# SiddhantSKarki/Vision-Transformer

Measured on AMD Instinct MI355X. Metric: images/sec fwd+bwd ViT-Base/16 224^2 bf16 (train step incl. AdamW); % MFMA roofline, higher is better.
Workload: dtype bf16; 1 GPU; ViT-Base/16 224x224 train step (fwd+CE+bwd+AdamW), batch 256/GPU; model=vit_base_patch16_224, global_batch=256, seq_len=197, parallelism=dp1

## Files before the change

include/vit_hip.h:

```cpp
#ifndef VIT_HIP_H
#define VIT_HIP_H

#include <stdint.h>

#ifdef __cplusplus
extern "C" {
#endif

#define VIT_ABI_VERSION 18

typedef enum { VIT_OK = 0, VIT_ERR_INVALID = 1, VIT_ERR_LAUNCH = 2 } vit_status;
typedef enum { VIT_F32 = 0, VIT_BF16 = 1, VIT_MASK4 = 2 } vit_dtype;

typedef enum { VIT_ACT_NONE = 0, VIT_ACT_RELU = 1, VIT_ACT_GELU = 2 } vit_act;

#define VIT_FLAG_SHARED_CUS 1

int vit_abi_version(void);
const char* vit_last_error(void);

int vit_set_option(const char* name, int64_t value);
int64_t vit_get_option(const char* name);

typedef struct vit_gemm_desc {
  const void* a;
  const void* b;
  void* c;
  int64_t lda, ldb, ldc;
  int64_t m, n, k;
  int32_t a_kcontig, b_kcontig;
  int32_t in_dtype;
  int32_t out_dtype;
  float alpha, beta;
  const float* bias;
  int32_t act;
  int32_t aux_dtype;
  const void* aux;
  int64_t ldaux;
  const void* res;
  int64_t ldres;
  int64_t res_rowmod;
  int32_t res_dtype;
  float dropout_p;
  uint32_t dropout_seed;
  int32_t split_k;
  int64_t out_group_rows, out_group_stride;
  void* workspace;
  int64_t workspace_bytes;
  float* colsum_part;
  void* mask_out;
  int64_t dropout_row_stride;
  int32_t flags;
  int64_t dropout_row0;
} vit_gemm_desc;

int64_t vit_gemm_workspace_bytes(const vit_gemm_desc* d);
int vit_gemm_split_k_hint(int64_t m, int64_t n, int64_t k, int in_dtype);
int vit_gemm(const vit_gemm_desc* d, void* stream);

#define VIT_DROP_PATH_MAX_LAYERS 64
int vit_drop_path_rows(float* out, uint32_t seed, int64_t L, int64_t B, int64_t T, const float* rates ,
                       void* stream);
int vit_gemm_rowscale(const vit_gemm_desc* d, const float* row_scale , void* stream);

#define VIT_EPI_BDR 3
#define VIT_EPI_SLAB 4
#define VIT_EPI_GENERAL 5
#define VIT_EPI_BDRS 8
int vit_gemm_kernel_choice(const vit_gemm_desc* d, const float* row_scale, int32_t* impl, int32_t* kind);

int vit_im2col(const void* x, int32_t x_dtype, void* cols, int32_t dtype, int64_t B, int64_t C, int64_t H,
               int64_t W, int64_t P, void* stream);
int vit_col2im(const void* cols, int32_t dtype, void* x, int32_t x_dtype, int64_t B, int64_t C, int64_t H, int64_t W,
               int64_t P, void* stream);
int vit_embed_cls(const float* cls, const float* pos, void* x0, int32_t dtype, int64_t B, int64_t T, int64_t D,
                  void* stream);

int vit_layernorm_fwd(const void* x, int64_t ldx, const float* gamma, const float* beta, void* y, int64_t ldy,
                      float* mean, float* rstd, int64_t rows, int64_t cols, float eps, int32_t dtype, void* stream);
int64_t vit_layernorm_bwd_parts(int64_t rows, int64_t cols);
int vit_layernorm_bwd(const void* dy, int64_t lddy, const void* x, int64_t ldx, const float* gamma,
                      const float* mean, const float* rstd, const void* dres, void* dx_out, void* drop_out,
                      float drop_p, uint32_t drop_seed, const void* drop_mask, float* partial, int32_t osum,
                      int64_t rows, int64_t cols, int32_t dtype, void* stream);

int vit_attn_fwd(const void* qkv, void* o, float* o32, float* lse, float* probs, int64_t B, int64_t T, int64_t H,
                 int64_t hd, float scale, int32_t dtype, int64_t max_wgs, void* stream);
int vit_attn_bwd_uses_o32(int64_t B, int64_t T, int64_t H, int64_t hd, int32_t dtype);
int64_t vit_attn_bwd_workspace_bytes(int64_t B, int64_t T, int64_t H, int64_t hd, int32_t dtype);
int vit_attn_bwd(const void* qkv, const void* o, const float* o32, const void* d_o, const float* lse, void* dqkv,
                 int64_t B, int64_t T, int64_t H, int64_t hd, float scale, int32_t dtype, void* workspace,
                 int32_t flags, void* stream);

int vit_attn_fwd_row0(const void* qkv, void* o, float* lse, int64_t B, int64_t T, int64_t H, int64_t hd, float scale,
                      int32_t dtype, void* stream);
int vit_attn_bwd_row0(const void* qkv, const void* d_o0, int64_t ldo, void* dqkv, int64_t B, int64_t T, int64_t H,
                      int64_t hd, float scale, int32_t dtype, void* stream);

int64_t vit_colsum_workspace_bytes(int64_t rows, int64_t cols);
int vit_colsum(const void* x, int64_t ldx, int32_t dtype, int64_t rows, int64_t cols, float* out, float alpha,
               float beta, void* workspace, void* stream);
int vit_colsum_finish(const float* part, int64_t nparts, int64_t cols, int32_t nsets, float* out0, float* out1,
                      float* out2, float beta, void* stream);
typedef struct {
  const float* part;
  int64_t nparts, cols;
  int32_t nsets;
  float* out[3];
  float beta;
} vit_colsum_job;
int vit_colsum_finish_batch(const vit_colsum_job* jobs, int32_t njobs, void* stream);
int vit_copy2d(const void* src, int64_t lds, int32_t src_dtype, void* dst, int64_t ldd, int32_t dst_dtype,
               int64_t rows, int64_t cols, int64_t src_group_rows, int64_t src_group_stride, float beta,
               void* stream);
int vit_dropout_bwd(const void* x, void* y, int32_t dtype, int64_t n, float p, uint32_t seed, float scale,
                    void* stream);
int vit_relu_bwd(const void* dy, const void* y, void* dx, int32_t dtype, int64_t n, void* stream);
// ... 80 lines not shown
```

vision-transformer_amd/VisionTransformer/_engine.py:

```python
from __future__ import annotations

import contextlib
import ctypes
import math
import weakref
from typing import NamedTuple, Optional

import torch
import torch.distributed as dist
from torch.optim.optimizer import register_optimizer_step_post_hook
from torch.utils.weak import WeakIdKeyDictionary

from . import _lib, _ops
from ._ops import ACT_NONE, ACT_RELU

SHADOWS = WeakIdKeyDictionary()


def shadow_of(p):
    return SHADOWS.get(p)


_ENGINE_OF = {}

# ... 15 lines not shown

DROPOUT_P = 0.2
LN_EPS = 1e-5
ALIGN = 64


def _hash_u32(seed, idx):
    x = (idx * 0x9E3779B1 + seed) & 0xFFFFFFFF
    x ^= x >> 16
    x = (x * 0x85EBCA6B) & 0xFFFFFFFF
    x ^= x >> 13
    x = (x * 0xC2B2AE35) & 0xFFFFFFFF
    x ^= x >> 16
    return x


def site_seed(base_seed, layer, site):
    return _hash_u32((base_seed * 0x632BE5AB + 0x1234567) & 0xFFFFFFFF, layer * 2 + site)


def dropout_seed(base_seed, rank=0):
    if rank == 0:
        return base_seed
    return _hash_u32((base_seed ^ 0x5BD1E995) & 0xFFFFFFFF, 0x27D4EB2F + rank) & 0x7FFFFFFF


def path_keep(base_seed, L, layer, site, B, p):
    thr = min(int(ctypes.c_float(p).value * 4294967296.0), 0xFFFFFFFF)
    s = site_seed(base_seed, L + layer, site)
    return torch.tensor([_hash_u32(s, b) >= thr for b in range(B)], dtype=torch.bool)


def _keep_scale(p):
    if p == 0.0:
        return DROPOUT_P, 1.0 / (1.0 - DROPOUT_P)
    keep = (1.0 - DROPOUT_P) * (1.0 - p)
    return 1.0 - keep, 1.0 / keep


class _Region:
    def __init__(self):
        self.size = 0
        self.items = []

    def add(self, name, numel):
        off = self.size
        self.items.append((name, off, numel))
        self.size = off + ((numel + ALIGN - 1) // ALIGN) * ALIGN
        return off


def split_k_for(m, n, k, dtype=torch.bfloat16):
    return int(_lib.load().vit_gemm_split_k_hint(m, n, k, _ops.dtype_code(dtype)))


def head_split_for(m, n, k):
    tiles = ((m + 63) // 64) * ((n + 63) // 64)
    nkt = (k + 31) // 32
    return max(1, min((1024 + tiles - 1) // tiles, nkt // 4, 32))


class Tape:
    __slots__ = ("B", "cols", "blocks", "z", "u", "gz", "zn", "mh", "rh", "seed", "training", "x_shape", "x_dtype",
                 "x_grad", "pruned", "row0", "path_rates")


BLOCK_REGIONS = ("qkv_w", "proj_w", "proj_b", "fc1_w", "fc1_b", "fc2_w", "fc2_b", "ln1_w", "ln1_b", "ln2_w", "ln2_b")


class BlockActs(NamedTuple):
    x_in: torch.Tensor
    a1: torch.Tensor
    m1: torch.Tensor
    r1: torch.Tensor
    qkv: torch.Tensor
    o: torch.Tensor
    o32: Optional[torch.Tensor]
    lse: torch.Tensor
    x_mid: torch.Tensor
    a2: torch.Tensor
    m2: torch.Tensor
    r2: torch.Tensor
    h: torch.Tensor
    hm: Optional[torch.Tensor]
    pm: Optional[torch.Tensor]
    fm: Optional[torch.Tensor]

    def images(self, b0, B, T):
        r0, R = b0 * T, B * T
        D = self.x_mid.shape[1]

        def rows(t):
            return None if t is None else t[r0:r0 + R]

        def bits(mask, n):
            if mask is None:
                return None
            off = (r0 // 4) * ((n + 3) // 4) * 4
            return mask[off:off + _ops.mask4_bytes(R, n)]

        s = self
        return BlockActs(x_in=rows(s.x_in), a1=rows(s.a1), m1=rows(s.m1), r1=rows(s.r1), qkv=rows(s.qkv), o=rows(s.o),
                         o32=rows(s.o32), lse=s.lse[b0:b0 + B], x_mid=rows(s.x_mid), a2=rows(s.a2), m2=rows(s.m2),
                         r2=rows(s.r2), h=rows(s.h), hm=bits(s.hm, 4 * D), pm=bits(s.pm, D), fm=bits(s.fm, D))


# ... 177 lines not shown
        self.stats["packs"] += 1

    def _token_rows(self, name, M, D, dt, T, dev):
        key = (name, M, D, dt, T, dev)
        buf = self._tok.get(key) if self._tok is not None else None
        if buf is None:
            if self._tok is None:
                self._tok = {}
            buf = self._tok[key] = torch.zeros(M, D, dtype=dt, device=dev)
        return buf

    def _workspace(self, nbytes, side=False):
        ws = self._ws[side]
        if ws is None or ws.numel() * 4 < nbytes:
            ws = self._ws[side] = torch.empty(max(nbytes // 4 + 1, 1 << 20), dtype=torch.float32, device=self.device)
        return ws

    def _split_ws(self, split, m, n, side=False):
        return self._workspace(split * m * n * 4, side) if split > 1 else None

    def _side_stream(self):
        if not self.concurrent_wgrad or self.device is None or self.device.type != "cuda":
            return None
        if self._wstream is None or self._wstream.device != self.device:
            self._wstream = torch.cuda.Stream(device=self.device)
        return self._wstream

    def _mark(self, fam, phase, flop=0.0, nbytes=0.0):
        h = self.profile_hook
        if h is not None:
            h(fam, phase, flop, nbytes)
        if self.trace_ranges:
            if phase == 0:
                torch.cuda.nvtx.range_push(fam)
            else:
                torch.cuda.nvtx.range_pop()

    def _wgrad(self, dy, x, out, m, n, k, ld_dy, ld_x, beta, side=None, fam=None, alpha=1.0):
        split = split_k_for(m, n, k, dy.dtype)
        ws = self._split_ws(split, m, n, side is not None)
        if side is not None:
            side.wait_stream(torch.cuda.current_stream(self.device))
        elif fam:
            self._mark(fam, 0, 2.0 * m * n * k, (m + n) * k * dy.element_size() + m * n * 4 * (1 + (beta != 0)))
        _ops.gemm(dy, x, out, m, n, k, ld_dy, ld_x, out.stride(0), a_kcontig=False, b_kcontig=False, beta=beta,
                  alpha=alpha, split_k=split, workspace=ws, stream=side)
        if side is not None:
            for t in (dy, x) if ws is None else (dy, x, ws):
                t.record_stream(side)
        elif fam:
            self._mark(fam, 1)

    def _gemm_rows(self, pr, a, b, c, m, n, k, lda, ldb, ldc, **kw):
        split = split_k_for(m, n, k, a.dtype) if pr else 1
        return _ops.gemm(a, b, c, m, n, k, lda, ldb, ldc, split_k=split, workspace=self._split_ws(split, m, n), **kw)

    def _head_gemm(self, a, b, c, m, n, k, lda, ldb, ldc, **kw):
        split = head_split_for(m, n, k)
        _ops.gemm(a, b, c, m, n, k, lda, ldb, ldc, split_k=split, workspace=self._split_ws(split, m, n), **kw)

    def _head_linear(self, x, w, bias):
        m, k = x.shape
        n = w.shape[0]
        y = torch.empty(m, n, dtype=x.dtype, device=x.device)
        self._head_gemm(x, w, y, m, n, k, x.stride(0), w.stride(0), n, bias=bias)
        return y

    def _attach_grads(self):
        views = [(p, gv) for p, gv in self.grad_views if p.requires_grad]
        live = [p.grad is not None and p.grad.data_ptr() == gv.data_ptr() for p, gv in views]
        if all(live):
            return 1.0
        if not any(p.grad is not None for p, _ in views):
            if not self.defer_grad_attach:
                for p, gv in views:
                    p.grad = gv
                return 0.0
            self._pending_views = views
            return 0.0
        for (p, gv), ok in zip(views, live):
            if not ok:
                if p.grad is not None:
                    gv.copy_(p.grad)
                else:
                    gv.zero_()
                p.grad = gv
        return 1.0

    def _attach_pending(self):
        views, self._pending_views = self._pending_views, None
        for p, gv in views or ():
            p.grad = gv

    def forward(self, x, training, save, want_probs=False):
        if not x.is_cuda:
            raise RuntimeError("VisionTransformer (HIP path) needs the input on a ROCm device; there is no CPU path")
        if x.dim() != 4 or x.shape[1] != self.C or x.shape[2] % self.P or x.shape[3] % self.P:
            raise RuntimeError(f"expected input [B, {self.C}, H, W] with H, W multiples of {self.P}, got "
                               f"{tuple(x.shape)}")
        B = x.shape[0]
        self.ensure_ready(x.device)
        if (x.shape[2] // self.P) * (x.shape[3] // self.P) != self.N:
            raise RuntimeError(f"image gives {(x.shape[2] // self.P) * (x.shape[3] // self.P)} patches but "
                               f"config.num_patches = {self.N} (pos_embd has {self.T} rows)")
        if B != self.params["cls"].shape[0]:
            raise RuntimeError(f"batch size {B} != config.batch_size {self.params['cls'].shape[0]} "
                               "(the CLS token parameter is batch-shaped)")
        x = x.contiguous()
        if x.dtype not in (torch.float32, torch.bfloat16):
            x = x.float()
        D, T, L, dt = self.D, self.T, self.L, self.dtype
# ... 508 lines not shown
```

vision-transformer_amd/VisionTransformer/_lib.py:

```python
import ctypes
import os

import torch

LIB_PATH = os.environ.get("VIT_HIP_LIB") or os.path.join(os.path.dirname(os.path.abspath(__file__)), "libvit_hip.so")
ABI_VERSION = 18

F32, BF16, MASK4 = 0, 1, 2
FLAG_SHARED_CUS = 1
ACT_NONE, ACT_RELU, ACT_GELU = 0, 1, 2


class GemmDesc(ctypes.Structure):
    _fields_ = [
        ("a", ctypes.c_void_p), ("b", ctypes.c_void_p), ("c", ctypes.c_void_p),
        ("lda", ctypes.c_int64), ("ldb", ctypes.c_int64), ("ldc", ctypes.c_int64),
        ("m", ctypes.c_int64), ("n", ctypes.c_int64), ("k", ctypes.c_int64),
        ("a_kcontig", ctypes.c_int32), ("b_kcontig", ctypes.c_int32),
        ("in_dtype", ctypes.c_int32), ("out_dtype", ctypes.c_int32),
        ("alpha", ctypes.c_float), ("beta", ctypes.c_float),
        ("bias", ctypes.c_void_p),
        ("act", ctypes.c_int32), ("aux_dtype", ctypes.c_int32),
        ("aux", ctypes.c_void_p), ("ldaux", ctypes.c_int64),
        ("res", ctypes.c_void_p), ("ldres", ctypes.c_int64), ("res_rowmod", ctypes.c_int64),
# ... 33 lines not shown

_P, _I64, _I32, _F, _U32 =ctypes.c_void_p, ctypes.c_int64, ctypes.c_int32, ctypes.c_float, ctypes.c_uint32

_SIGS = {
    "vit_abi_version": (ctypes.c_int, []),
    "vit_last_error": (ctypes.c_char_p, []),
    "vit_set_option": (ctypes.c_int, [ctypes.c_char_p, _I64]),
    "vit_get_option": (_I64, [ctypes.c_char_p]),
    "vit_gemm_workspace_bytes": (_I64, [ctypes.POINTER(GemmDesc)]),
    "vit_gemm": (ctypes.c_int, [ctypes.POINTER(GemmDesc), _P]),
    "vit_gemm_split_k_hint": (ctypes.c_int, [_I64, _I64, _I64, _I32]),
    "vit_im2col": (ctypes.c_int, [_P, _I32, _P, _I32, _I64, _I64, _I64, _I64, _I64, _P]),
    "vit_col2im": (ctypes.c_int, [_P, _I32, _P, _I32, _I64, _I64, _I64, _I64, _I64, _P]),
    "vit_embed_cls": (ctypes.c_int, [_P, _P, _P, _I32, _I64, _I64, _I64, _P]),
    "vit_layernorm_fwd": (ctypes.c_int, [_P, _I64, _P, _P, _P, _I64, _P, _P, _I64, _I64, _F, _I32, _P]),
    "vit_layernorm_bwd_parts": (_I64, [_I64, _I64]),
    "vit_layernorm_bwd": (ctypes.c_int, [_P, _I64, _P, _I64, _P, _P, _P, _P, _P, _P, _F, _U32, _P, _P, _I32, _I64,
                                         _I64, _I32, _P]),
    "vit_attn_fwd": (ctypes.c_int, [_P, _P, _P, _P, _P, _I64, _I64, _I64, _I64, _F, _I32, _I64, _P]),
    "vit_attn_bwd_uses_o32": (ctypes.c_int, [_I64, _I64, _I64, _I64, _I32]),
    "vit_attn_bwd_workspace_bytes": (_I64, [_I64, _I64, _I64, _I64, _I32]),
    "vit_attn_bwd": (ctypes.c_int, [_P, _P, _P, _P, _P, _P, _I64, _I64, _I64, _I64, _F, _I32, _P, _I32, _P]),
    "vit_attn_fwd_row0": (ctypes.c_int, [_P, _P, _P, _I64, _I64, _I64, _I64, _F, _I32, _P]),
    "vit_attn_bwd_row0": (ctypes.c_int, [_P, _P, _I64, _P, _I64, _I64, _I64, _I64, _F, _I32, _P]),
    "vit_colsum_workspace_bytes": (_I64, [_I64, _I64]),
    "vit_colsum": (ctypes.c_int, [_P, _I64, _I32, _I64, _I64, _P, _F, _F, _P, _P]),
    "vit_colsum_finish": (ctypes.c_int, [_P, _I64, _I64, _I32, _P, _P, _P, _F, _P]),
    "vit_colsum_finish_batch": (ctypes.c_int, [ctypes.POINTER(ColsumJob), _I32, _P]),
    "vit_copy2d": (ctypes.c_int, [_P, _I64, _I32, _P, _I64, _I32, _I64, _I64, _I64, _I64, _F, _P]),
    "vit_dropout_bwd": (ctypes.c_int, [_P, _P, _I32, _I64, _F, _U32, _F, _P]),
    "vit_mask4_apply": (ctypes.c_int, [_P, _I64, _I32, _P, _I64, _I32, _P, _I64, _I64, _F, _P]),
    "vit_relu_bwd": (ctypes.c_int, [_P, _P, _P, _I32, _I64, _P]),
    "vit_gelu_fwd": (ctypes.c_int, [_P, _P, _I64, _P]),
    "vit_gelu_bwd": (ctypes.c_int, [_P, _P, _P, _I64, _P]),
    "vit_softmax_xent": (ctypes.c_int, [_P, _P, _I64, _I64, _P, _P, _P, _P]),
    "vit_resize_ksize": (ctypes.c_int, [_I64, _I64]),
    "vit_resize_workspace_bytes": (_I64, [_I64, _I64, _I64, _I64]),
    "vit_resize_to_tensor": (ctypes.c_int, [_P, _P, _I64, _I64, _I64, _I64, _P, _I32, _P, _I64, _P]),
    "vit_adamw": (ctypes.c_int, [_P, _I64, _F, _F, _F, _F, _F, _F, _F, _F, _I32, _P]),
    "vit_pack": (ctypes.c_int, [_P, _I64, _I32, _P]),
    "vit_grad_sumsq": (ctypes.c_int, [_P, _I64, _F, _P, _P]),
    "vit_grad_clip_finish": (ctypes.c_int, [_P, _I64, _F, _P, _P]),
    "vit_adamw_clipped": (ctypes.c_int, [_P, _I64, _F, _F, _F, _F, _F, _F, _F, _F, _I32, _P, _P]),
    "vit_adamw_ema": (ctypes.c_int, [_P, _P, _I64, _F, _F, _F, _F, _F, _F, _F, _F, _I32, _F, _P, _P]),
    "vit_ema_swap": (ctypes.c_int, [_P, _P, _I64, _I32, _P]),
    "vit_softmax_xent_mixed": (ctypes.c_int, [_P, _P, _P, _P, _F, _I64, _I64, _P, _P, _P, _P]),
    "vit_mix_batch": (ctypes.c_int, [_P, _P, _I32, _I64, _I64, _I64, _I64, _P, _P]),
    "vit_augment_workspace_bytes": (_I64, [_I64, _I64, _I64, _I64]),
    "vit_augment_to_tensor": (ctypes.c_int, [_P, _P, _P, _I64, _I64, _I64, _I64, _P, _P, _F, _P, _I32, _P, _I64, _P]),
    "vit_drop_path_rows": (ctypes.c_int, [_P, _U32, _I64, _I64, _I64, ctypes.POINTER(ctypes.c_float), _P]),
    "vit_gemm_rowscale": (ctypes.c_int, [ctypes.POINTER(GemmDesc), _P, _P]),
    "vit_gemm_kernel_choice": (ctypes.c_int, [ctypes.POINTER(GemmDesc), _P, ctypes.POINTER(_I32),
                                              ctypes.POINTER(_I32)]),
    "vit_lamb_moments": (ctypes.c_int, [_P, _I64, _F, _F, _F, _F, _F, _F, _F, _P, _P, _P]),
    "vit_lamb_trust": (ctypes.c_int, [_P, _P, _I64, _I32, _I32, _P, _P, _P]),
    "vit_lamb_update": (ctypes.c_int, [_P, _P, _P, _P, _I64, _F, _F, _F, _F, _F, _I32, _F, _P, _P]),
}

EPI_BDR, EPI_SLAB, EPI_GENERAL, EPI_BDRS = 3, 4, 5, 8

DROP_PATH_MAX_LAYERS = 64

EXPORTED_SYMBOLS = tuple(_SIGS.keys())

_lib = None


class HipLibraryError(RuntimeError):
    pass


def load():
    global _lib
    if _lib is not None:
        return _lib
    if not os.path.exists(LIB_PATH):
        raise HipLibraryError(f"{LIB_PATH} not found: build it with `make -C vision-transformer_amd/csrc` or "
                              "`python -c 'import __graft_entry__ as g; g.build()'` (there is no CPU fallback)")
    lib = ctypes.CDLL(LIB_PATH, mode=ctypes.RTLD_GLOBAL)
    for name, (res, args) in _SIGS.items():
        fn = getattr(lib, name)
        fn.restype = res
        fn.argtypes = args
    v = lib.vit_abi_version()
    if v != ABI_VERSION:
        raise HipLibraryError(f"libvit_hip ABI version {v} != expected {ABI_VERSION}")
    _lib = lib
    return lib


def check(rc, what):
    if rc != 0:
        msg = load().vit_last_error().decode(errors="replace")
        raise RuntimeError(f"{what} failed (status {rc}): {msg}")


def call(name, *args):
    lib = load()
    check(getattr(lib, name)(*args), name)


def set_option(name, value):
    lib = load()
    prev = lib.vit_get_option(name.encode())
    check(lib.vit_set_option(name.encode(), int(value)), f"vit_set_option({name!r})")
    return prev


def get_option(name):
    v = load().vit_get_option(name.encode())
    if v == -(1 << 63):
        raise KeyError(f"unknown libvit_hip option {name!r}")
# ... 16 lines not shown
```

vision-transformer_amd/csrc/vit_common.h:

```cpp
#pragma once

#include <hip/hip_runtime.h>
#include <hip/hip_bf16.h>
#include <stdint.h>
#include <algorithm>

#include "../../include/vit_hip.h"

typedef uint16_t bf16_t;
typedef __bf16 bf16x8_t __attribute__((ext_vector_type(8)));
typedef short s16x8 __attribute__((ext_vector_type(8)));
typedef short s16x4 __attribute__((ext_vector_type(4)));
typedef float f32x4 __attribute__((ext_vector_type(4)));
typedef float f32x16 __attribute__((ext_vector_type(16)));

#define VIT_DEV __device__ __forceinline__

VIT_DEV int remat(int x) {
  asm volatile("" : "+v"(x));
  return x;
}

VIT_DEV void item_bh(int64_t item, int64_t H, int64_t& b, int64_t& h) {
  const int u = (int)item, hh = (int)H;
// ... 40 lines not shown
  x.x = (uint32_t)f2bf(v[0]) | ((uint32_t)f2bf(v[1]) << 16);
  x.y = (uint32_t)f2bf(v[2]) | ((uint32_t)f2bf(v[3]) << 16);
  *reinterpret_cast<uint2*>(p) = x;
}

VIT_DEV uint32_t vit_hash_u32(uint32_t seed, uint32_t idx) {
  uint32_t x = idx * 0x9E3779B1u + seed;
  x ^= x >> 16; x *= 0x85EBCA6Bu;
  x ^= x >> 13; x *= 0xC2B2AE35u;
  x ^= x >> 16;
  return x;
}
VIT_DEV int64_t mask4_byte(int64_t i, int64_t j, int64_t n) { return (((i >> 2) * ((n + 3) >> 2)) + (j >> 2)) * 4 + (i & 3); }

static inline uint32_t vit_drop_threshold(float p) {
  double t = (double)p * 4294967296.0;
  return t >= 4294967295.0 ? 0xffffffffu : (uint32_t)t;
}

VIT_DEV float wave_sum(float v) {
#pragma unroll
  for (int o = 32; o > 0; o >>= 1) v += __shfl_xor(v, o, 64);
  return v;
}
VIT_DEV float wave_max(float v) {
#pragma unroll
  for (int o = 32; o > 0; o >>= 1) v = fmaxf(v, __shfl_xor(v, o, 64));
  return v;
}

VIT_DEV float gelu_erf(float x) { return 0.5f * x * (1.0f + erff(x * 0.70710678118654752f)); }
VIT_DEV float gelu_erf_grad(float x) {
  const float cdf = 0.5f * (1.0f + erff(x * 0.70710678118654752f));
  const float pdf = 0.39894228040143268f * __expf(-0.5f * x * x);
  return cdf + x * pdf;
}

namespace vit {
void set_error(const char* fmt, ...);
int check_launch(const char* what);
void colsum_parts_launch(const void* x, int64_t ldx, int dtype, int64_t rows, int64_t cols, int64_t rows_per_chunk,
                         float* part, hipStream_t s);
}

#define VIT_OPTIONS(X)                              \
  X(OPT_GEMM_IMPL, "gemm_impl", 0)                  \
  X(OPT_GEMM_TAIL, "gemm_tail", 0)                  \
  X(OPT_GEMM_TAIL_MIN_KT, "gemm_tail_min_kt", 40)   \
  X(OPT_SPLITK_MIN_KT, "splitk_min_kt", 0)          \
  X(OPT_SPLITK_ROUNDS, "splitk_rounds", 1)          \
  X(OPT_GEMM_GROUP_M, "gemm_group_m", 0)            \
  X(OPT_GEMM_EPI_GENERAL, "gemm_epi_general", 0)    \
  X(OPT_GEMM_PERSIST, "gemm_persist", 1)            \
  X(OPT_ATTN_FWD_SPLIT, "attn_fwd_split", 0)        \
  X(OPT_ATTN_BWD_SPLIT, "attn_bwd_split", 0)        \
  X(OPT_ATTN_FWD_GRID, "attn_fwd_grid", 0)          \
  X(OPT_ATTN_BWD_GRID, "attn_bwd_grid", 0)          \
  X(OPT_LN16, "ln16", 1)                            \
  X(OPT_LN_AL, "ln_al", 1)                          \
  X(OPT_AUGMENT_PATH, "augment_path", 0)
namespace vit {
enum Opt : int {
#define X(ENUM, NAME, DEF) ENUM,
  VIT_OPTIONS(X)
#undef X
  OPT_COUNT
};
int64_t opt(Opt o);
}

static inline int64_t vit_cu_count() {
  static int cache[64] = {0};
  int dev = 0;
  if (hipGetDevice(&dev) != hipSuccess || dev < 0 || dev >= 64) return 256;
  if (cache[dev] == 0) {
    int n = 0;
    if (hipDeviceGetAttribute(&n, hipDeviceAttributeMultiprocessorCount, dev) != hipSuccess || n <= 0) n = 256;
    cache[dev] = n;
  }
  return cache[dev];
}

#define VIT_REQUIRE(cond, ...)                 \
  do {                                         \
    if (!(cond)) {                             \
      vit::set_error(__VA_ARGS__);             \
      return VIT_ERR_INVALID;                  \
    }                                          \
  } while (0)

#define VIT_STREAM(s) (reinterpret_cast<hipStream_t>(s))
```

vision-transformer_amd/csrc/vit_gemm.hip:

```cpp
#include "vit_common.h"

namespace {

struct EpiParams {
  void* c;
  int64_t ldc, m, n;
  float alpha, beta;
  const float* bias;
  int act;
  const void* aux;
  int64_t ldaux;
  int aux_dtype;
  const void* res;
  int64_t ldres, res_rowmod;
  int res_dtype;
  uint32_t drop_thr, seed;
  float drop_scale;
  int use_drop;
  int64_t grp, grp_stride;
  int vec;
  int vec8;
  float* csum;
  int64_t row0;
  uint8_t* mask_out;
// ... 1084 lines not shown
      const float a_op = Ws[2 * kk + (lane >> 5)][wn * 32 + (lane & 31)];
      const float b_op = Xs[2 * kk + (lane >> 5)][wm * 32 + (lane & 31)];
      acc = __builtin_amdgcn_mfma_f32_32x32x2f32(a_op, b_op, acc, 0, 0, 0);
    }
    __syncthreads();
  }
#pragma unroll
  for (int grp = 0; grp < 4; ++grp) {
    const int64_t i = i0 + wm * 32 + (lane & 31);
    const int64_t j = j0 + wn * 32 + 8 * grp + 4 * (lane >> 5);
    float v[4] = {acc[4 * grp], acc[4 * grp + 1], acc[4 * grp + 2], acc[4 * grp + 3]};
    if (g.ws) slab_store4(g.ws + (int64_t)blockIdx.y * g.M * g.N, g.M, g.N, i, j, v);
    else epilogue4<TO>(e, i, j, v);
  }
}

template <class TO>
__global__ __launch_bounds__(256) void splitk_reduce_kernel(const float* __restrict__ ws, int64_t M, int64_t N,
                                                            int splits, EpiParams e) {
  const int64_t nq = (N + 3) / 4;
  const int64_t total = M * nq;
  for (int64_t t = blockIdx.x * (int64_t)blockDim.x + threadIdx.x; t < total;
       t += (int64_t)gridDim.x * blockDim.x) {
    const int64_t i = t / nq, j = (t % nq) * 4;
    float v[4] = {0.f, 0.f, 0.f, 0.f};
    int z = 0;
    if ((N & 3) == 0) {
      for (; z + 4 <= splits; z += 4) {
        f32x4 x[4];
#pragma unroll
        for (int u = 0; u < 4; ++u)
          x[u] = __builtin_nontemporal_load(reinterpret_cast<const f32x4*>(ws + (int64_t)(z + u) * M * N + i * N + j));
#pragma unroll
        for (int u = 0; u < 4; ++u)
#pragma unroll
          for (int r = 0; r < 4; ++r) v[r] += x[u][r];
      }
    }
    for (; z < splits; ++z) {
      const float* p = ws + (int64_t)z * M * N + i * N + j;
      if ((N & 3) == 0) {
        float x[4];
        ld4<float>(p, x);
#pragma unroll
        for (int r = 0; r < 4; ++r) v[r] += x[r];
      } else {
        for (int r = 0; r < 4 && j + r < N; ++r) v[r] += p[r];
      }
    }
    epilogue4<TO>(e, i, j, v);
  }
}

bool aligned(const void* p, int a) { return p == nullptr || (((uintptr_t)p) % a) == 0; }

int gemm_impl_env() {
  const int64_t v = vit::opt(vit::OPT_GEMM_IMPL);
  return (v == 1 || v == 2 || v == 4) ? (int)v : 0;
}

int gemm_impl(int64_t m, int64_t n) {
  const int forced = gemm_impl_env();
  if (forced) return forced;
  return (m >= 256 && n >= 256) ? 4 : 2;
}

int tail_split(const vit_gemm_desc* d, int64_t* m_main) {
  *m_main = d->m;
  if (d->split_k > 1 || d->in_dtype != VIT_BF16 || d->k % BK != 0 || d->m <= 0 || d->n <= 0) return 1;
  if (gemm_impl(d->m, d->n) != 4 || d->out_group_rows != 0 || d->res_rowmod != 0) return 1;
  if (!vit::opt(vit::OPT_GEMM_TAIL)) return 1;
  const int64_t tn = (d->n + 255) / 256, tm = (d->m + 255) / 256, nkt = d->k / BK;
  const int64_t rounds = tm * tn / 256;
  const int64_t min_kt = vit::opt(vit::OPT_GEMM_TAIL_MIN_KT);
  if (rounds < 1 || nkt < min_kt) return 1;
  const int64_t mr = rounds * 256 / tn;
  const int64_t tail = (tm - mr) * tn;
  if (tail <= 0 || 2 * tail > 256) return 1;
  const int64_t sk = std::min<int64_t>(std::min<int64_t>(256 / tail, nkt / 4), 8);
  if (sk < 2) return 1;
  *m_main = mr * 256;
  return (int)sk;
}

int gemm_validate(const vit_gemm_desc* d) {
  VIT_REQUIRE(d != nullptr, "vit_gemm: null descriptor");
  VIT_REQUIRE(d->a && d->b && d->c, "vit_gemm: null operand pointer");
  VIT_REQUIRE(!d->colsum_part || d->out_group_rows == 0, "vit_gemm: colsum_part needs ungrouped output rows");
  VIT_REQUIRE(d->m > 0 && d->n > 0 && d->k > 0, "vit_gemm: bad shape m=%lld n=%lld k=%lld", (long long)d->m,
              (long long)d->n, (long long)d->k);
  VIT_REQUIRE(d->in_dtype == VIT_F32 || d->in_dtype == VIT_BF16, "vit_gemm: bad in_dtype %d", d->in_dtype);
  VIT_REQUIRE(d->out_dtype == VIT_F32 || d->out_dtype == VIT_BF16, "vit_gemm: bad out_dtype %d", d->out_dtype);
  VIT_REQUIRE(d->beta == 0.f || d->out_dtype == VIT_F32, "vit_gemm: beta requires f32 output");
  VIT_REQUIRE(!d->aux || d->aux_dtype == VIT_F32 || d->aux_dtype == VIT_BF16 || d->aux_dtype == VIT_MASK4,
              "vit_gemm: bad aux_dtype %d", d->aux_dtype);
  VIT_REQUIRE(!d->mask_out || d->out_group_rows == 0, "vit_gemm: mask_out needs ungrouped output rows");
  VIT_REQUIRE(!d->mask_out || aligned(d->mask_out, 4), "vit_gemm: mask_out must be 4-B aligned");
  VIT_REQUIRE(!d->aux || d->aux_dtype != VIT_MASK4 || aligned(d->aux, 4), "vit_gemm: mask4 aux must be 4-B aligned");
  VIT_REQUIRE(d->dropout_p >= 0.f && d->dropout_p < 1.f, "vit_gemm: dropout_p out of range");
  if (d->in_dtype == VIT_BF16) {
    const bool akc = d->a_kcontig != 0, bkc = d->b_kcontig != 0;
    VIT_REQUIRE(aligned(d->a, 16) && aligned(d->b, 16), "vit_gemm(bf16): operands must be 16-B aligned");
    VIT_REQUIRE(d->lda % 8 == 0 && d->ldb % 8 == 0, "vit_gemm(bf16): lda/ldb must be multiples of 8");
    VIT_REQUIRE(akc ? d->k % 8 == 0 : d->m % 8 == 0, "vit_gemm(bf16): A contiguous dim must be a multiple of 8");
    VIT_REQUIRE(bkc ? d->k % 8 == 0 : d->n % 8 == 0, "vit_gemm(bf16): B contiguous dim must be a multiple of 8");
    VIT_REQUIRE(akc || !bkc, "vit_gemm(bf16): layout (A rowstrided, B kcontig) is not provided");
// ... 54 lines not shown
  else if (e.grp > 0 && e.res_rowmod > 0 && e.bias && e.res && e.res_dtype == VIT_F32 && e.act == VIT_ACT_NONE &&
           !e.aux && !e.use_drop && e.m < 0x7fffffffLL)
    kind = EPI_PATCH;
  return kind_has(kind, akc, bkc) ? kind : EPI_GENERAL;
}

struct Launch {
  GemmArgs g;
  EpiParams e;
  int64_t a_bytes, b_bytes;
  dim3 grid;
  hipStream_t s;
};

template <bool AKC, bool BKC, class TO, int KIND>
void launch_v4(const Launch& L) {
  gemm_bf16_v4<AKC, BKC, TO, KIND><<<L.grid, 512, 0, L.s>>>(L.g, L.e, L.a_bytes, L.b_bytes);
}

template <bool AKC, bool BKC>
void launch_bf16(int impl, int kind, bool to_bf, const Launch& L) {
  if (impl == 4) {
    if (!to_bf) {
      if (kind == EPI_SLAB) launch_v4<AKC, BKC, float, EPI_SLAB>(L);
      else launch_v4<AKC, BKC, float, EPI_GENERAL>(L);
      return;
    }
    switch (kind) {
      case EPI_PLAIN: return launch_v4<AKC, BKC, bf16_t, EPI_PLAIN>(L);
      case EPI_BIAS_ACT: return launch_v4<AKC, BKC, bf16_t, EPI_BIAS_ACT>(L);
      case EPI_BDR: return launch_v4<AKC, BKC, bf16_t, EPI_BDR>(L);
      case EPI_BDRS: return launch_v4<AKC, BKC, bf16_t, EPI_BDRS>(L);
      case EPI_AUX: return launch_v4<AKC, BKC, bf16_t, EPI_AUX>(L);
      case EPI_AUXM: return launch_v4<AKC, BKC, bf16_t, EPI_AUXM>(L);
      case EPI_PATCH: return launch_v4<AKC, BKC, bf16_t, EPI_PATCH>(L);
      default: return launch_v4<AKC, BKC, bf16_t, EPI_GENERAL>(L);
    }
  }
  if (impl == 2) {
    if (to_bf) gemm_bf16_v2<AKC, BKC, bf16_t><<<L.grid, 256, 0, L.s>>>(L.g, L.e, L.a_bytes, L.b_bytes);
    else gemm_bf16_v2<AKC, BKC, float><<<L.grid, 256, 0, L.s>>>(L.g, L.e, L.a_bytes, L.b_bytes);
  } else {
    if (to_bf) gemm_bf16_kernel<AKC, BKC, bf16_t><<<L.grid, 256, 0, L.s>>>(L.g, L.e);
    else gemm_bf16_kernel<AKC, BKC, float><<<L.grid, 256, 0, L.s>>>(L.g, L.e);
  }
}

template <bool AKC, bool BKC>
void launch_f32(bool to_bf, const Launch& L) {
  if (to_bf) gemm_f32_kernel<AKC, BKC, bf16_t><<<L.grid, 256, 0, L.s>>>(L.g, L.e);
  else gemm_f32_kernel<AKC, BKC, float><<<L.grid, 256, 0, L.s>>>(L.g, L.e);
}

}


extern "C" int64_t vit_gemm_workspace_bytes(const vit_gemm_desc* d) {
  if (!d) return 0;
  if (d->split_k > 1) return (int64_t)d->split_k * d->m * d->n * (int64_t)sizeof(float);
  int64_t m_main = 0;
  const int sk = tail_split(d, &m_main);
  return sk > 1 ? (int64_t)sk * (d->m - m_main) * d->n * (int64_t)sizeof(float) : 0;
}

extern "C" int vit_gemm_split_k_hint(int64_t m, int64_t n, int64_t k, int in_dtype) {
  if (m <= 0 || n <= 0 || k <= 0) return 1;
  if (in_dtype == VIT_BF16 && k % BK == 0 && gemm_impl(m, n) == 4) {
    const int64_t tiles = ((m + 255) / 256) * ((n + 255) / 256);
    const int64_t min_env = vit::opt(vit::OPT_SPLITK_MIN_KT);
    const int64_t nkt = k / BK, min_kt = min_env > 0 ? min_env : (nkt >= 16 ? 4 : 1);
    const int64_t rounds = std::max<int64_t>(1, vit::opt(vit::OPT_SPLITK_ROUNDS));
    const int64_t s = std::min<int64_t>(std::min<int64_t>(256 * rounds / tiles, nkt / min_kt), 64);
    return (int)std::max<int64_t>(1, s);
  }
  const int64_t tiles = ((m + 127) / 128) * ((n + 127) / 128);
  const int64_t nkt = (k + 63) / 64;
  const int64_t s = std::min<int64_t>(std::min<int64_t>((1024 + tiles - 1) / tiles, std::max<int64_t>(1, nkt / 8)), 32);
  return (int)std::max<int64_t>(1, s);
}


struct Plan {
  int impl, kind;
  int64_t a_bytes, b_bytes;
};
static Plan gemm_plan(const vit_gemm_desc* d, const EpiParams& e) {
  Plan p{0, EPI_GENERAL, 0, 0};
  if (d->in_dtype != VIT_BF16) return p;
  const bool akc = d->a_kcontig != 0, bkc = d->b_kcontig != 0;
  p.a_bytes = (akc ? (d->m - 1) * d->lda + d->k : (d->k - 1) * d->lda + d->m) * 2;
  p.b_bytes = (bkc ? (d->n - 1) * d->ldb + d->k : (d->k - 1) * d->ldb + d->n) * 2;
  const bool dma_ok = d->k % BK == 0 && p.a_bytes < 0x7fffffffLL && p.b_bytes < 0x7fffffffLL;
  p.impl = dma_ok ? gemm_impl(d->m, d->n) : 1;
  if (p.impl == 4) p.kind = v4_kind(e, akc, bkc, d->out_dtype == VIT_BF16, d->split_k > 1 ? d->split_k : 1);
  return p;
}

static int gemm_run(const vit_gemm_desc* d, int64_t row0, const float* row_scale, void* stream) {
  const int split = d->split_k > 1 ? d->split_k : 1;
  const bool in_bf = d->in_dtype == VIT_BF16, out_bf = d->out_dtype == VIT_BF16;
  const bool to_bf = out_bf && split == 1;
  const bool akc = d->a_kcontig != 0, bkc = d->b_kcontig != 0;
  Launch L{};
  L.e = make_epi(d, row0, row_scale);
  L.s = VIT_STREAM(stream);
  GemmArgs& g = L.g;
  g.a = d->a; g.b = d->b; g.lda = d->lda; g.ldb = d->ldb; g.M = d->m; g.N = d->n; g.K = d->k;
  if (split > 1) {
    VIT_REQUIRE(d->workspace && d->workspace_bytes >= vit_gemm_workspace_bytes(d),
                "vit_gemm: split_k=%d needs %lld workspace bytes", split, (long long)vit_gemm_workspace_bytes(d));
    g.ws = (float*)d->workspace;
  }

  const Plan plan = gemm_plan(d, L.e);
  const int impl = plan.impl, kind = plan.kind;
  int64_t tile = FBM, bk = FBK;
  if (in_bf) {
    L.a_bytes = plan.a_bytes;
    L.b_bytes = plan.b_bytes;
    tile = impl == 4 ? 256 : BM;
    bk = BK;
    g.nitems = ((d->m + 255) / 256) * ((d->n + 255) / 256) * split;
    VIT_REQUIRE(g.nitems < (1LL << 31), "vit_gemm: %lld tiles exceed the 2^31 work items of one launch",
                (long long)g.nitems);
  }
  g.tiles_m = (d->m + tile - 1) / tile;
  g.tiles_n = (d->n + tile - 1) / tile;
  g.kt_per_split = ((d->k + bk - 1) / bk + split - 1) / split;
  L.grid = dim3((unsigned)(g.tiles_m * g.tiles_n), (unsigned)split);
  bool cs_fused = false;
  if (impl == 4) {
    const bool wide = kind != EPI_SLAB && kind != EPI_GENERAL;
    cs_fused = wide && d->colsum_part;
    if (cs_fused) L.e.csum = d->colsum_part;
    const int64_t gopt = vit::opt(vit::OPT_GEMM_GROUP_M);
    g.group_m = gopt > 0 ? gopt : (g.tiles_n >= 16 ? 8 : 1);
    const bool persist = wide && L.e.act != VIT_ACT_GELU && !(d->flags & VIT_FLAG_SHARED_CUS) &&
                         vit::opt(vit::OPT_GEMM_PERSIST);
    L.grid = dim3((unsigned)(persist ? std::min<int64_t>(g.nitems, vit_cu_count()) : g.nitems), 1u);
  }

  if (in_bf) {
    if (akc && bkc) launch_bf16<true, true>(impl, kind, to_bf, L);
    else if (akc) launch_bf16<true, false>(impl, kind, to_bf, L);
    else launch_bf16<false, false>(impl, kind, to_bf, L);
  } else if (akc) {
    if (bkc) launch_f32<true, true>(to_bf, L);
    else launch_f32<true, false>(to_bf, L);
  } else {
    if (bkc) launch_f32<false, true>(to_bf, L);
    else launch_f32<false, false>(to_bf, L);
  }
  if (split > 1) {
    const int64_t total = d->m * ((d->n + 3) / 4);
    const int64_t blocks = std::min<int64_t>((total + 255) / 256, 4096);
    if (out_bf) splitk_reduce_kernel<bf16_t><<<(unsigned)blocks, 256, 0, L.s>>>(g.ws, d->m, d->n, split, L.e);
    else splitk_reduce_kernel<float><<<(unsigned)blocks, 256, 0, L.s>>>(g.ws, d->m, d->n, split, L.e);
  }
  if (d->colsum_part && !cs_fused)
    vit::colsum_parts_launch(d->c, d->ldc, d->out_dtype, d->m, d->n, 256, d->colsum_part, L.s);
  return vit::check_launch("vit_gemm");
}

static int gemm_entry(const vit_gemm_desc* d, const float* row_scale, void* stream) {
  if (const int rc = gemm_validate(d)) return rc;
  VIT_REQUIRE(aligned(row_scale, 4), "vit_gemm_rowscale: row_scale must be 4-B aligned");
  int64_t m_main = 0;
  const int sk = tail_split(d, &m_main);
  if (sk <= 1 || !d->workspace || d->workspace_bytes < vit_gemm_workspace_bytes(d))
    return gemm_run(d, d->dropout_row0, row_scale, stream);
  vit_gemm_desc dm = *d;
  dm.m = m_main;
  if (const int rc = gemm_run(&dm, d->dropout_row0, row_scale, stream)) return rc;
  auto esz = [](int32_t t) { return t == VIT_BF16 ? (int64_t)2 : (int64_t)4; };
  const int64_t r = m_main;
  vit_gemm_desc dt = *d;
  dt.a = (const char*)d->a + (d->a_kcontig ? r * d->lda : r) * 2;
  dt.c = (char*)d->c + r * d->ldc * esz(d->out_dtype);
  const int64_t mask_off = (r / 4) * ((d->n + 3) / 4) * 4;
  if (d->aux) dt.aux = (const char*)d->aux + (d->aux_dtype == VIT_MASK4 ? mask_off : r * d->ldaux * esz(d->aux_dtype));
  if (d->mask_out) dt.mask_out = (char*)d->mask_out + mask_off;
  if (d->res) dt.res = (const char*)d->res + r * d->ldres * esz(d->res_dtype);
  if (d->colsum_part) dt.colsum_part = d->colsum_part + (r / 256) * d->n;
  dt.m = d->m - r;
  dt.split_k = sk;
  return gemm_run(&dt, d->dropout_row0 + r, row_scale, stream);
}

extern "C" int vit_gemm(const vit_gemm_desc* d, void* stream) { return gemm_entry(d, nullptr, stream); }

static_assert(EPI_BDR == VIT_EPI_BDR && EPI_BDRS == VIT_EPI_BDRS && EPI_GENERAL == VIT_EPI_GENERAL &&
              EPI_SLAB == VIT_EPI_SLAB, "vit_hip.h names the epilogue kinds vit_gemm_kernel_choice reports");

extern "C" int vit_gemm_kernel_choice(const vit_gemm_desc* d, const float* row_scale, int32_t* impl, int32_t* kind) {
  if (const int rc = gemm_validate(d)) return rc;
  VIT_REQUIRE(impl && kind, "vit_gemm_kernel_choice: null output pointer");
  int64_t m_main = 0;
  vit_gemm_desc dm = *d;
  if (tail_split(d, &m_main) > 1 && d->workspace && d->workspace_bytes >= vit_gemm_workspace_bytes(d)) dm.m = m_main;
  const Plan p = gemm_plan(&dm, make_epi(&dm, d->dropout_row0, row_scale));
  *impl = p.impl;
  *kind = p.kind;
  return VIT_OK;
}

extern "C" int vit_gemm_rowscale(const vit_gemm_desc* d, const float* row_scale, void* stream) {
  return gemm_entry(d, row_scale, stream);
}
```

Baseline: 8329 images/s.

## Add few-row GEMM kernel with intra-block K split for small-M shapes

```diff
diff --git a/include/vit_hip.h b/include/vit_hip.h
--- a/include/vit_hip.h
+++ b/include/vit_hip.h
@@ -56,6 +56,7 @@
 
 int64_t vit_gemm_workspace_bytes(const vit_gemm_desc* d);
 int vit_gemm_split_k_hint(int64_t m, int64_t n, int64_t k, int in_dtype);
+int vit_gemm_few_rows(int64_t m, int64_t n, int64_t k, int in_dtype);
 int vit_gemm(const vit_gemm_desc* d, void* stream);
 
 #define VIT_DROP_PATH_MAX_LAYERS 64
@@ -63,6 +64,7 @@
                        void* stream);
 int vit_gemm_rowscale(const vit_gemm_desc* d, const float* row_scale , void* stream);
 
+#define VIT_GEMM_IMPL_FEWROW 6
 #define VIT_EPI_BDR 3
 #define VIT_EPI_SLAB 4
 #define VIT_EPI_GENERAL 5
diff --git a/vision-transformer_amd/VisionTransformer/_engine.py b/vision-transformer_amd/VisionTransformer/_engine.py
--- a/vision-transformer_amd/VisionTransformer/_engine.py
+++ b/vision-transformer_amd/VisionTransformer/_engine.py
@@ -91,6 +91,10 @@
 
 def split_k_for(m, n, k, dtype=torch.bfloat16):
     return int(_lib.load().vit_gemm_split_k_hint(m, n, k, _ops.dtype_code(dtype)))
+
+
+def few_rows(m, n, k, dtype=torch.bfloat16):
+    return bool(_lib.load().vit_gemm_few_rows(m, n, k, _ops.dtype_code(dtype)))
 
 
 def head_split_for(m, n, k):
@@ -374,11 +378,11 @@
             self._mark(fam, 1)
 
     def _gemm_rows(self, pr, a, b, c, m, n, k, lda, ldb, ldc, **kw):
-        split = split_k_for(m, n, k, a.dtype) if pr else 1
+        split = split_k_for(m, n, k, a.dtype) if pr and not few_rows(m, n, k, a.dtype) else 1
         return _ops.gemm(a, b, c, m, n, k, lda, ldb, ldc, split_k=split, workspace=self._split_ws(split, m, n), **kw)
 
     def _head_gemm(self, a, b, c, m, n, k, lda, ldb, ldc, **kw):
-        split = head_split_for(m, n, k)
+        split = 1 if few_rows(m, n, k, a.dtype) else head_split_for(m, n, k)
         _ops.gemm(a, b, c, m, n, k, lda, ldb, ldc, split_k=split, workspace=self._split_ws(split, m, n), **kw)
 
     def _head_linear(self, x, w, bias):
diff --git a/vision-transformer_amd/VisionTransformer/_lib.py b/vision-transformer_amd/VisionTransformer/_lib.py
--- a/vision-transformer_amd/VisionTransformer/_lib.py
+++ b/vision-transformer_amd/VisionTransformer/_lib.py
@@ -109,12 +109,14 @@
     "vit_gemm_rowscale": (ctypes.c_int, [ctypes.POINTER(GemmDesc), _P, _P]),
     "vit_gemm_kernel_choice": (ctypes.c_int, [ctypes.POINTER(GemmDesc), _P, ctypes.POINTER(_I32),
                                               ctypes.POINTER(_I32)]),
+    "vit_gemm_few_rows": (ctypes.c_int, [_I64, _I64, _I64, _I32]),
     "vit_lamb_moments": (ctypes.c_int, [_P, _I64, _F, _F, _F, _F, _F, _F, _F, _P, _P, _P]),
     "vit_lamb_trust": (ctypes.c_int, [_P, _P, _I64, _I32, _I32, _P, _P, _P]),
     "vit_lamb_update": (ctypes.c_int, [_P, _P, _P, _P, _I64, _F, _F, _F, _F, _F, _I32, _F, _P, _P]),
 }
 
 EPI_BDR, EPI_SLAB, EPI_GENERAL, EPI_BDRS = 3, 4, 5, 8
+GEMM_IMPL_FEWROW = 6
 
 DROP_PATH_MAX_LAYERS = 64
 
diff --git a/vision-transformer_amd/csrc/vit_common.h b/vision-transformer_amd/csrc/vit_common.h
--- a/vision-transformer_amd/csrc/vit_common.h
+++ b/vision-transformer_amd/csrc/vit_common.h
@@ -116,6 +116,7 @@
   X(OPT_GEMM_GROUP_M, "gemm_group_m", 0)            \
   X(OPT_GEMM_EPI_GENERAL, "gemm_epi_general", 0)    \
   X(OPT_GEMM_PERSIST, "gemm_persist", 1)            \
+  X(OPT_GEMM_FEWROW, "gemm_fewrow", 1)              \
   X(OPT_ATTN_FWD_SPLIT, "attn_fwd_split", 0)        \
   X(OPT_ATTN_BWD_SPLIT, "attn_bwd_split", 0)        \
   X(OPT_ATTN_FWD_GRID, "attn_fwd_grid", 0)          \
diff --git a/vision-transformer_amd/csrc/vit_gemm.hip b/vision-transformer_amd/csrc/vit_gemm.hip
--- a/vision-transformer_amd/csrc/vit_gemm.hip
+++ b/vision-transformer_amd/csrc/vit_gemm.hip
@@ -1160,6 +1160,217 @@
   }
 }
 
+constexpr int FR_T = 32;
+constexpr int FR_U = 8;
+constexpr int FR_UB = 4;
+constexpr int FR_LDW = 40;
+
+struct FewArgs {
+  const void* a;
+  const void* b;
+  int64_t lda, ldb;
+  int M, N, K;
+  int tiles_m, tiles_n;
+  int avec, bvec;
+};
+
+VIT_DEV bool few_tile(const FewArgs& g, int& tm, int& tn) {
+  const int b = blockIdx.x, q = b >> 3;
+  tm = q % g.tiles_m;
+  tn = (q / g.tiles_m) * 8 + (b & 7);
+  return tn < g.tiles_n;
+}
+
+VIT_DEV f32x4 few_reduce(f32x4* part, const f32x4 (&acc)[4], int wave, int lane) {
+#pragma unroll
+  for (int q = 0; q < 4; ++q) part[(wave * 4 + q) * 64 + lane] = acc[q];
+  __syncthreads();
+  f32x4 s = part[(0 * 4 + wave) * 64 + lane];
+#pragma unroll
+  for (int w = 1; w < 4; ++w) s += part[(w * 4 + wave) * 64 + lane];
+  return s;
+}
+
+template <int U>
+struct FewBf16Batch {
+  uint4 a[U][2], b[U][2];
+};
+
+template <bool BKC, int U>
+VIT_DEV void few_load_bf16(const bf16_t* const (&pa)[2], const bf16_t* const (&pb)[2], bool bcol_ok, int64_t ldb,
+                           int K, int k0, int lane, FewBf16Batch<U>& r) {
+#pragma unroll
+  for (int u = 0; u < U; ++u) {
+    const int k = k0 + u * 32;
+    const int kl = k + 8 * (lane >> 4);
+#pragma unroll
+    for (int x = 0; x < 2; ++x) {
+      r.a[u][x] = make_uint4(0u, 0u, 0u, 0u);
+      if (kl < K) r.a[u][x] = *reinterpret_cast<const uint4*>(pa[x] + kl);
+    }
+#pragma unroll
+    for (int y = 0; y < 2; ++y) {
+      r.b[u][y] = make_uint4(0u, 0u, 0u, 0u);
+      if (BKC) {
+        if (kl < K) r.b[u][y] = *reinterpret_cast<const uint4*>(pb[y] + kl);
+      } else {
+        const int kr = k + 16 * y + (lane >> 2);
+        if (kr < K && bcol_ok) r.b[u][y] = *reinterpret_cast<const uint4*>(pb[0] + (int64_t)kr * ldb);
+      }
+    }
+  }
+}
+
+template <bool BKC, int U>
+VIT_DEV void few_mma_bf16(f32x4 (&acc)[4], const FewBf16Batch<U>& r, bf16_t* img, int lane) {
+  f32x4 t[4];
+#pragma unroll
+  for (int q = 0; q < 4; ++q) t[q] = f32x4{0.f, 0.f, 0.f, 0.f};
+#pragma unroll
+  for (int u = 0; u < U; ++u) {
+    bf16x8_t bf[2];
+    if (BKC) {
+      bf[0] = __builtin_bit_cast(bf16x8_t, r.b[u][0]);
+      bf[1] = __builtin_bit_cast(bf16x8_t, r.b[u][1]);
+    } else {
+      __builtin_amdgcn_fence(__ATOMIC_RELEASE, "wavefront");
+      *reinterpret_cast<uint4*>(img + (lane >> 2) * FR_LDW + 8 * (lane & 3)) = r.b[u][0];
+      *reinterpret_cast<uint4*>(img + (16 + (lane >> 2)) * FR_LDW + 8 * (lane & 3)) = r.b[u][1];
+      __builtin_amdgcn_fence(__ATOMIC_ACQ_REL, "wavefront");
+#pragma unroll
+      for (int y = 0; y < 2; ++y) {
+        s16x8 v;
+#pragma unroll
+        for (int t = 0; t < 8; ++t) v[t] = (short)img[(8 * (lane >> 4) + t) * FR_LDW + y * 16 + (lane & 15)];
+        bf[y] = __builtin_bit_cast(bf16x8_t, v);
+      }
+    }
+#pragma unroll
+    for (int x = 0; x < 2; ++x)
+#pragma unroll
+      for (int y = 0; y < 2; ++y)
+        t[x * 2 + y] = __builtin_amdgcn_mfma_f32_16x16x32_bf16(bf[y], __builtin_bit_cast(bf16x8_t, r.a[u][x]),
+                                                               t[x * 2 + y], 0, 0, 0);
+  }
+#pragma unroll
+  for (int q = 0; q < 4; ++q) acc[q] += t[q];
+}
+
+template <bool BKC, class TO, int U>
+__global__ __launch_bounds__(256) void gemm_fewrow_bf16(FewArgs g, EpiParams e) {
+  __shared__ __attribute__((aligned(16))) f32x4 part[4 * 4 * 64];
+  __shared__ __attribute__((aligned(16))) bf16_t img[BKC ? 8 : 4 * 32 * FR_LDW];
+  const int tid = threadIdx.x, lane = tid & 63, wave = tid >> 6;
+  int tm, tn;
+  if (!few_tile(g, tm, tn)) return;
+  const int i0 = tm * FR_T, j0 = tn * FR_T;
+  const bf16_t* A = (const bf16_t*)g.a;
+  const bf16_t* B = (const bf16_t*)g.b;
+  const bf16_t* pa[2];
+  const bf16_t* pb[2];
+#pragma unroll
+  for (int x = 0; x < 2; ++x) pa[x] = A + (int64_t)min(i0 + x * 16 + (lane & 15), g.M - 1) * g.lda;
+  bool bcol_ok = true;
+  if (BKC) {
+#pragma unroll
+    for (int y = 0; y < 2; ++y) pb[y] = B + (int64_t)min(j0 + y * 16 + (lane & 15), g.N - 1) * g.ldb;
+  } else {
+    const int col = j0 + 8 * (lane & 3);
+    bcol_ok = col < g.N;
+    pb[0] = pb[1] = B + (bcol_ok ? col : 0);
+  }
+  f32x4 acc[4];
+#pragma unroll
+  for (int q = 0; q < 4; ++q) acc[q] = f32x4{0.f, 0.f, 0.f, 0.f};
+  constexpr int KB = 32 * U;
+  bf16_t* my_img = img + (BKC ? 0 : wave * 32 * FR_LDW);
+  FewBf16Batch<U> r0, r1, r2;
+  few_load_bf16<BKC, U>(pa, pb, bcol_ok, g.ldb, g.K, wave * KB, lane, r0);
+  few_load_bf16<BKC, U>(pa, pb, bcol_ok, g.ldb, g.K, wave * KB + 4 * KB, lane, r1);
+  for (int k = wave * KB; k < g.K; k += 12 * KB) {
+    few_load_bf16<BKC, U>(pa, pb, bcol_ok, g.ldb, g.K, k + 8 * KB, lane, r2);
+    few_mma_bf16<BKC, U>(acc, r0, my_img, lane);
+    if (k + 4 * KB >= g.K) break;
+    few_load_bf16<BKC, U>(pa, pb, bcol_ok, g.ldb, g.K, k + 12 * KB, lane, r0);
+    few_mma_bf16<BKC, U>(acc, r1, my_img, lane);
+    if (k + 8 * KB >= g.K) break;
+    few_load_bf16<BKC, U>(pa, pb, bcol_ok, g.ldb, g.K, k + 16 * KB, lane, r1);
+    few_mma_bf16<BKC, U>(acc, r2, my_img, lane);
+  }
+  const f32x4 s = few_reduce(part, acc, wave, lane);
+  const int x = wave >> 1, y = wave & 1;
+  float v[4] = {s[0], s[1], s[2], s[3]};
+  epilogue4<TO>(e, i0 + x * 16 + (lane & 15), j0 + y * 16 + 4 * (lane >> 4), v);
+}
+
+struct FewF32Batch {
+  f32x4 a[FR_U], b[FR_U];
+};
+
+template <bool KC>
+VIT_DEV f32x4 few_ld4_f32(const float* p, int64_t ld, int vec, int K, int k) {
+  f32x4 v = {0.f, 0.f, 0.f, 0.f};
+  if (KC) {
+    if (vec && k + 3 < K) return *reinterpret_cast<const f32x4*>(p + k);
+#pragma unroll
+    for (int t = 0; t < 4; ++t)
+      if (k + t < K) v[t] = p[k + t];
+  } else {
+#pragma unroll
+    for (int t = 0; t < 4; ++t)
+      if (k + t < K) v[t] = p[(int64_t)(k + t) * ld];
+  }
+  return v;
+}
+
+template <bool BKC>
+VIT_DEV void few_load_f32(const float* pa, const float* pb, const FewArgs& g, int k0, int lane, FewF32Batch& r) {
+#pragma unroll
+  for (int u = 0; u < FR_U; ++u) {
+    const int k = k0 + u * 8 + 4 * (lane >> 5);
+    r.a[u] = few_ld4_f32<true>(pa, g.lda, g.avec, g.K, k);
+    r.b[u] = few_ld4_f32<BKC>(pb, g.ldb, g.bvec, g.K, k);
+  }
+}
+
+VIT_DEV void few_mma_f32(f32x16& acc, const FewF32Batch& r) {
+  f32x16 s = {};
+#pragma unroll
+  for (int u = 0; u < FR_U; ++u)
+#pragma unroll
+    for (int t = 0; t < 4; ++t) s = __builtin_amdgcn_mfma_f32_32x32x2f32(r.b[u][t], r.a[u][t], s, 0, 0, 0);
+  acc += s;
+}
+
+template <bool BKC, class TO>
+__global__ __launch_bounds__(256) void gemm_fewrow_f32(FewArgs g, EpiParams e) {
+  __shared__ __attribute__((aligned(16))) f32x4 part[4 * 4 * 64];
+  const int tid = threadIdx.x, lane = tid & 63, wave = tid >> 6;
+  int tm, tn;
+  if (!few_tile(g, tm, tn)) return;
+  const int i0 = tm * FR_T, j0 = tn * FR_T;
+  const float* pa = (const float*)g.a + (int64_t)min(i0 + (lane & 31), g.M - 1) * g.lda;
+  const int jb = min(j0 + (lane & 31), g.N - 1);
+  const float* pb = (const float*)g.b + (BKC ? (int64_t)jb * g.ldb : (int64_t)jb);
+  f32x16 acc = {};
+  constexpr int KB = 8 * FR_U;
+  FewF32Batch r0, r1;
+  few_load_f32<BKC>(pa, pb, g, wave * KB, lane, r0);
+  for (int k = wave * KB; k < g.K; k += 8 * KB) {
+    few_load_f32<BKC>(pa, pb, g, k + 4 * KB, lane, r1);
+    few_mma_f32(acc, r0);
+    if (k + 4 * KB >= g.K) break;
+    few_load_f32<BKC>(pa, pb, g, k + 8 * KB, lane, r0);
+    few_mma_f32(acc, r1);
+  }
+  f32x4 a4[4];
+#pragma unroll
+  for (int q = 0; q < 4; ++q) a4[q] = f32x4{acc[4 * q], acc[4 * q + 1], acc[4 * q + 2], acc[4 * q + 3]};
+  const f32x4 s = few_reduce(part, a4, wave, lane);
+  float v[4] = {s[0], s[1], s[2], s[3]};
+  epilogue4<TO>(e, i0 + (lane & 31), j0 + 8 * wave + 4 * (lane >> 5), v);
+}
+
 bool aligned(const void* p, int a) { return p == nullptr || (((uintptr_t)p) % a) == 0; }
 
 int gemm_impl_env() {
@@ -1320,6 +1531,50 @@
   else gemm_f32_kernel<AKC, BKC, float><<<L.grid, 256, 0, L.s>>>(L.g, L.e);
 }
 
+constexpr int FEW_IMPL = VIT_GEMM_IMPL_FEWROW;
+constexpr int64_t FEW_MAX_M = 256, FEW_MIN_K = 256;
+
+bool fewrow_shape(int64_t m, int64_t n, int64_t k, int in_dtype) {
+  const int64_t o = vit::opt(vit::OPT_GEMM_FEWROW);
+  if (o <= 0 || gemm_impl_env() != 0 || m <= 0 || m > FEW_MAX_M || n <= 0 || k <= 0) return false;
+  if (n >= (1LL << 30) || k >= (1LL << 30)) return false;
+  return o >= 2 || (k >= FEW_MIN_K && in_dtype == VIT_BF16);
+}
+
+bool fewrow_takes(const vit_gemm_desc* d) {
+  return d->split_k <= 1 && d->a_kcontig != 0 && fewrow_shape(d->m, d->n, d->k, d->in_dtype);
+}
+
+template <bool BKC>
+void launch_fewrow(bool in_bf, bool out_bf, const FewArgs& g, const EpiParams& e, unsigned grid, hipStream_t s) {
+  if (in_bf) {
+    if (out_bf) gemm_fewrow_bf16<BKC, bf16_t, FR_UB><<<grid, 256, 0, s>>>(g, e);
+    else gemm_fewrow_bf16<BKC, float, FR_UB><<<grid, 256, 0, s>>>(g, e);
+  } else {
+    if (out_bf) gemm_fewrow_f32<BKC, bf16_t><<<grid, 256, 0, s>>>(g, e);
+    else gemm_fewrow_f32<BKC, float><<<grid, 256, 0, s>>>(g, e);
+  }
+}
+
+int fewrow_run(const vit_gemm_desc* d, const float* row_scale, void* stream) {
+  FewArgs g{};
+  g.a = d->a; g.b = d->b; g.lda = d->lda; g.ldb = d->ldb;
+  g.M = (int)d->m; g.N = (int)d->n; g.K = (int)d->k;
+  g.tiles_m = (g.M + FR_T - 1) / FR_T;
+  g.tiles_n = (g.N + FR_T - 1) / FR_T;
+  g.avec = d->lda % 4 == 0 && aligned(d->a, 16);
+  g.bvec = d->ldb % 4 == 0 && aligned(d->b, 16);
+  const EpiParams e = make_epi(d, d->dropout_row0, row_scale);
+  const unsigned grid = (unsigned)(8 * g.tiles_m * ((g.tiles_n + 7) / 8));
+  hipStream_t s = VIT_STREAM(stream);
+  const bool in_bf = d->in_dtype == VIT_BF16, out_bf = d->out_dtype == VIT_BF16;
+  if (d->b_kcontig) launch_fewrow<true>(in_bf, out_bf, g, e, grid, s);
+  else launch_fewrow<false>(in_bf, out_bf, g, e, grid, s);
+  if (d->colsum_part)
+    vit::colsum_parts_launch(d->c, d->ldc, d->out_dtype, d->m, d->n, 256, d->colsum_part, s);
+  return vit::check_launch("vit_gemm");
+}
+
 }
 
 
@@ -1348,12 +1603,20 @@
 }
 
 
+extern "C" int vit_gemm_few_rows(int64_t m, int64_t n, int64_t k, int in_dtype) {
+  return fewrow_shape(m, n, k, in_dtype) ? 1 : 0;
+}
+
 struct Plan {
   int impl, kind;
   int64_t a_bytes, b_bytes;
 };
 static Plan gemm_plan(const vit_gemm_desc* d, const EpiParams& e) {
   Plan p{0, EPI_GENERAL, 0, 0};
+  if (fewrow_takes(d)) {
+    p.impl = FEW_IMPL;
+    return p;
+  }
   if (d->in_dtype != VIT_BF16) return p;
   const bool akc = d->a_kcontig != 0, bkc = d->b_kcontig != 0;
   p.a_bytes = (akc ? (d->m - 1) * d->lda + d->k : (d->k - 1) * d->lda + d->m) * 2;
@@ -1433,6 +1696,7 @@
 static int gemm_entry(const vit_gemm_desc* d, const float* row_scale, void* stream) {
   if (const int rc = gemm_validate(d)) return rc;
   VIT_REQUIRE(aligned(row_scale, 4), "vit_gemm_rowscale: row_scale must be 4-B aligned");
+  if (fewrow_takes(d)) return fewrow_run(d, row_scale, stream);
   int64_t m_main = 0;
   const int sk = tail_split(d, &m_main);
   if (sk <= 1 || !d->workspace || d->workspace_bytes < vit_gemm_workspace_bytes(d))
```

Result: no change. 8349 images/s, median of 6 (+0.2%).
